# LewisClifton/Deep-Super-Resolution

Hardware: AMD Instinct MI355X
Metric: HR Mpixels/sec x4 GAN train step; PSNR delta vs reference (higher is better)
Workload: dtype bf16; 1 GPU; gan_x4: full GAN step x4 (G + D + VGG19 perceptual), batch 32/GPU, 128x128->512x512; global_batch=32, parallelism=dp1

## Files before the change

### deep-super-resolution_amd/csrc/conv_wgrad_tile.hip

```cpp
#include "dsr_common.h"
#include "dsr_kernels.h"

__device__ __forceinline__ s16x4 tr_read(const unsigned char* p) {
  return __builtin_amdgcn_ds_read_tr16_b64_v4i16((__attribute__((address_space(3))) s16x4*)(p));
}
__device__ __forceinline__ U4 tr_frag(const unsigned char* base, int p1, int p2, int chunk, int within) {
  s16x4 lo = tr_read(base + p1 * 128 + ((chunk ^ (p1 & 7)) << 4) + within);
  s16x4 hi = tr_read(base + p2 * 128 + ((chunk ^ (p2 & 7)) << 4) + within);
  return __builtin_bit_cast(U4, __builtin_shufflevector(lo, hi, 0, 1, 2, 3, 4, 5, 6, 7));
}

template <int DT, int KH, int KW, int S>
__global__ __launch_bounds__(256, 2) void conv_wgrad_tile_kernel(const WgradTileArgs a) {
  constexpr int R = (S == 1) ? 4 : 2;
  constexpr int HR = (R - 1) * S + KH, HC = 31 * S + KW;
  constexpr int NT = KH * KW;
  __shared__ __attribute__((aligned(16))) unsigned char sX[HR * HC * 128];
  __shared__ __attribute__((aligned(16))) unsigned char sY[R * 32 * 128];

  const int tid = threadIdx.x, lane = tid & 63, wave = __builtin_amdgcn_readfirstlane(tid >> 6);
  const int wr = wave >> 1, wc = wave & 1;
  const int g = lane >> 4, l16 = lane & 15, q4 = l16 >> 2, cc = 4 * (l16 & 3);
  const int pair = blockIdx.x;
  const int co0 = (pair / a.tiles_ci) * 64, ci0 = (pair % a.tiles_ci) * 64;
  const unsigned short* __restrict__ X = reinterpret_cast<const unsigned short*>(a.x);
  const unsigned short* __restrict__ DY = reinterpret_cast<const unsigned short*>(a.dy);

  f32x4 acc[NT][2][2];
#pragma unroll
  for (int t = 0; t < NT; ++t)
#pragma unroll
    for (int i = 0; i < 2; ++i)
#pragma unroll
      for (int j = 0; j < 2; ++j) acc[t][i][j] = f32x4{0.f, 0.f, 0.f, 0.f};

  const int c = tid & 7, pbase = tid >> 3;
  const bool yc_ok = (co0 + c * 8) < a.CoutP, xc_ok = (ci0 + c * 8) < a.CinP;
  int t_end = (blockIdx.y + 1) * a.tiles_per_block;
  if (t_end > a.ntiles) t_end = a.ntiles;
  const int per_img = a.tiles_y * a.tiles_x;

  for (int t = blockIdx.y * a.tiles_per_block; t < t_end; ++t) {
    const int n = t / per_img;
    const int rem = t - n * per_img;
    const int oy0 = (rem / a.tiles_x) * R, ox0 = (rem % a.tiles_x) * 32;
    __syncthreads();
#pragma unroll
    for (int i = 0; i < R * 32 * 8 / 256; ++i) {
      const int p = pbase + 32 * i;
      const int oy = oy0 + (p >> 5), ox = ox0 + (p & 31);
      const bool ok = yc_ok && oy < a.OH && ox < a.OW;
      U4 v = load16_or_zero(DY, ((size_t)(n * a.OH + oy) * a.OW + ox) * a.CoutP + co0 + c * 8, ok);
      *reinterpret_cast<U4*>(sY + p * 128 + ((c ^ (p & 7)) << 4)) = v;
    }
    {
      constexpr int NV = (HR * HC + 31) / 32;
      U4 v[NV];
#pragma unroll
      for (int u = 0; u < NV; ++u) {
        const int q = pbase + 32 * u;
        const int hr = q / HC, hc = q - hr * HC;
        bool ok = xc_ok && q < HR * HC;
        const int iy = pad_index(oy0 * S + hr - a.pad, a.IH, a.pad_mode, ok);
        const int ix = pad_index(ox0 * S + hc - a.pad, a.IW, a.pad_mode, ok);
        v[u] = load16_or_zero(X, ((size_t)(n * a.IH + iy) * a.IW + ix) * a.CinP + ci0 + c * 8, ok);
      }
#pragma unroll
      for (int u = 0; u < NV; ++u) {
        const int q = pbase + 32 * u;
        if (q < HR * HC) *reinterpret_cast<U4*>(sX + q * 128 + ((c ^ (q & 7)) << 4)) = v[u];
      }
    }
    __syncthreads();
#pragma unroll 1
    for (int r = 0; r < R; ++r) {
      U4 fa[2];
#pragma unroll
      for (int i = 0; i < 2; ++i) {
        const int ch = wr * 32 + i * 16 + cc;
        fa[i] = tr_frag(sY, r * 32 + 4 * g + q4, r * 32 + 16 + 4 * g + q4, ch >> 3, (ch & 7) * 2);
      }
#pragma unroll
      for (int kh = 0; kh < KH; ++kh)
#pragma unroll
        for (int kw = 0; kw < KW; ++kw) {
          const int qb = (r * S + kh) * HC + kw;
          const int q1 = qb + (4 * g + q4) * S, q2 = qb + (16 + 4 * g + q4) * S;
          U4 fb[2];
#pragma unroll
          for (int j = 0; j < 2; ++j) {
            const int ch = wc * 32 + j * 16 + cc;
            fb[j] = tr_frag(sX, q1, q2, ch >> 3, (ch & 7) * 2);
          }
#pragma unroll
          for (int i = 0; i < 2; ++i)
#pragma unroll
            for (int j = 0; j < 2; ++j) acc[kh * KW + kw][i][j] = mfma16<DT>(fa[i], fb[j], acc[kh * KW + kw][i][j]);
        }
    }
  }

  float* P = a.partial + (size_t)blockIdx.y * NT * a.CoutP * a.CinP;
#pragma unroll
  for (int t = 0; t < NT; ++t)
#pragma unroll
    for (int i = 0; i < 2; ++i)
#pragma unroll
      for (int j = 0; j < 2; ++j)
#pragma unroll
        for (int r = 0; r < 4; ++r) {
          const int co = co0 + wr * 32 + i * 16 + 4 * g + r, ci = ci0 + wc * 32 + j * 16 + l16;
          if (co < a.CoutP && ci < a.CinP) P[((size_t)t * a.CoutP + co) * a.CinP + ci] = acc[t][i][j][r];
        }
}

template <int DT>
__device__ __forceinline__ void conv_wgrad_dma_body(const WgradTileArgs& a, const int pair, const int ychunk) {
  constexpr int R = 2, HC = 40, HR = R + 2;
  constexpr int XB = HR * HC * 128, YB = R * 32 * 128, STAGE = XB + YB;
  __shared__ __attribute__((aligned(16))) unsigned char smem[2 * STAGE];

  const int tid = threadIdx.x, lane = tid & 63, wave = __builtin_amdgcn_readfirstlane(tid >> 6);
  const int g = lane >> 4, l16 = lane & 15, q4 = l16 >> 2, cc = 4 * (l16 & 3);
  const int co0 = (pair / a.tiles_ci) * 64, ci0 = (pair % a.tiles_ci) * 64;

  f32x4 acc[9][4];
#pragma unroll
  for (int t = 0; t < 9; ++t)
#pragma unroll
    for (int i = 0; i < 4; ++i) acc[t][i] = f32x4{0.f, 0.f, 0.f, 0.f};

  const int lp = 4 * g + q4;
  int offA[4], offB[3];
#pragma unroll
  for (int i = 0; i < 4; ++i) {
    const int ch = i * 16 + cc;
    offA[i] = XB + lp * 128 + (((ch >> 3) ^ (lp & 7)) << 4) + (ch & 7) * 2;
  }
#pragma unroll
  for (int kw = 0; kw < 3; ++kw) {
    const int ch = wave * 16 + cc;
    offB[kw] = lp * 128 + (((ch >> 3) ^ ((kw + lp) & 7)) << 4) + (ch & 7) * 2;
  }

  const int chunk = (tid & 7) ^ ((tid >> 3) & 7), pb = tid >> 3;
  const bool yc_ok = (co0 + chunk * 8) < a.CoutP, xc_ok = (ci0 + chunk * 8) < a.CinP;
  const BufSrd xrsrc = make_srd(const_cast<void*>(a.x), a.x_bytes);
  const BufSrd yrsrc = make_srd(const_cast<void*>(a.dy), a.dy_bytes);
  constexpr unsigned OOB = 0xFFFFFFF0u;
  typedef __attribute__((address_space(3))) void* lds_ptr;
  const int per_img = a.tiles_y * a.tiles_x;
  constexpr int NX = (HR * HC) / 32, NY = (R * 32) / 32;
  constexpr int FAR = 0x7FFFFF00;
  int xpart[NX], ypart[NY];
  unsigned hc_pack = 0;
#pragma unroll
  for (int u = 0; u < NX; ++u) {
    const int q = pb + 32 * u;
    const int hr = q / HC, hc = q - hr * HC;
    xpart[u] = (xc_ok && hc < 34) ? ((hr * a.IW + hc) * a.CinP + ci0 + chunk * 8) * 2 : FAR;
    hc_pack |= (unsigned)hc << (6 * u);
  }
#pragma unroll
  for (int u = 0; u < NY; ++u) {
    const int p = pb + 32 * u;
    ypart[u] = yc_ok ? (((p >> 5) * a.OW + (p & 31)) * a.CoutP + co0 + chunk * 8) * 2 : FAR;
  }
  const unsigned ximg = (unsigned)(a.IH * a.IW * a.CinP * 2), yimg = (unsigned)(a.OH * a.OW * a.CoutP * 2);
  const bool fast = a.pad_mode == DSR_PAD_ZERO;
  struct TileXY {
    int n, ty, tx;
  };
  auto dma = [&](const TileXY& tc, int buf) {
    const int n = tc.n;
    const int oy0 = tc.ty * R, ox0 = tc.tx * 32;
    unsigned char* st = smem + buf * STAGE;
    if (fast) {
      const BufSrd xr = make_srd(const_cast<unsigned char*>(reinterpret_cast<const unsigned char*>(a.x)) + (size_t)n * ximg, ximg);
      const BufSrd yr = make_srd(const_cast<unsigned char*>(reinterpret_cast<const unsigned char*>(a.dy)) + (size_t)n * yimg, yimg);
      const int xs = ((oy0 - a.pad) * a.IW + ox0 - a.pad) * a.CinP * 2;
      const int ys = (oy0 * a.OW + ox0) * a.CoutP * 2;
      unsigned char* dx = st + 8 * wave * 128;
      if (ox0 - a.pad >= 0 && ox0 - a.pad + 34 <= a.IW) {
#pragma unroll
        for (int u = 0; u < NX; ++u)
          lds_dma16(xr, dx + 32 * u * 128, (unsigned)(xpart[u] + xs));
      } else {
#pragma unroll
        for (int u = 0; u < NX; ++u) {
          const int ix = ox0 - a.pad + (int)((hc_pack >> (6 * u)) & 63);
          lds_dma16(xr, dx + 32 * u * 128, (unsigned)ix < (unsigned)a.IW ? (unsigned)(xpart[u] + xs) : OOB);
        }
      }
      if (ox0 + 32 <= a.OW) {
#pragma unroll
        for (int u = 0; u < NY; ++u)
          lds_dma16(yr, dx + XB + 32 * u * 128, (unsigned)(ypart[u] + ys));
      } else {
#pragma unroll
        for (int u = 0; u < NY; ++u)
          lds_dma16(yr, dx + XB + 32 * u * 128, ox0 + (pb & 31) < a.OW ? (unsigned)(ypart[u] + ys) : OOB);
      }
      return;
    }
#pragma unroll
    for (int u = 0; u < (HR * HC) / 32; ++u) {
      const int q = pb + 32 * u;
      const int hr = q / HC, hc = q - hr * HC;
      bool ok = xc_ok && hc < 34;
      const int iy = pad_index(oy0 + hr - a.pad, a.IH, a.pad_mode, ok);
      const int ix = pad_index(ox0 + hc - a.pad, a.IW, a.pad_mode, ok);
      lds_dma16(xrsrc, st + (32 * u + 8 * wave) * 128, ok ? (unsigned)((((n * a.IH + iy) * a.IW + ix) * a.CinP + ci0 + chunk * 8) * 2) : OOB);
    }
#pragma unroll
    for (int u = 0; u < (R * 32) / 32; ++u) {
      const int p = pb + 32 * u;
      const int oy = oy0 + (p >> 5), ox = ox0 + (p & 31);
      const bool ok = yc_ok && oy < a.OH && ox < a.OW;
      lds_dma16(yrsrc, st + XB + (32 * u + 8 * wave) * 128, ok ? (unsigned)((((n * a.OH + oy) * a.OW + ox) * a.CoutP + co0 + chunk * 8) * 2) : OOB);
    }
  };
  auto next_tile = [&](TileXY c) {
    if (++c.tx == a.tiles_x) {
      c.tx = 0;
      if (++c.ty == a.tiles_y) {
        c.ty = 0;
        ++c.n;
      }
    }
    return c;
  };

  int t = ychunk * a.tiles_per_block;
  int t_end = t + a.tiles_per_block;
  if (t_end > a.ntiles) t_end = a.ntiles;
  TileXY nxt;
  nxt.n = t / per_img;
  nxt.ty = (t - nxt.n * per_img) / a.tiles_x;
  nxt.tx = t - nxt.n * per_img - nxt.ty * a.tiles_x;
  __builtin_amdgcn_s_setprio(1);
  if (t < t_end) dma(nxt, 0);
  int buf = 0;
  for (; t < t_end; ++t, buf ^= 1) {
    asm volatile("s_waitcnt vmcnt(0)" ::: "memory");
    __builtin_amdgcn_s_barrier();
    asm volatile("" ::: "memory");
    nxt = next_tile(nxt);
    if (t + 1 < t_end) dma(nxt, buf ^ 1);
    __builtin_amdgcn_s_setprio(0);
    const unsigned char* st = smem + buf * STAGE;
    auto frag = [&](int off) {
      const s16x4 lo = tr_read(st + off);
      const s16x4 hi = tr_read(st + off + 2048);
      return __builtin_bit_cast(U4, __builtin_shufflevector(lo, hi, 0, 1, 2, 3, 4, 5, 6, 7));
    };
    constexpr int NU = 3 * HR;
    auto load_b = [&](int u) {
      const int kw = u / HR, h = u - kw * HR;
      return frag(offB[kw] + (h * HC + kw) * 128);
    };
    U4 fa[R][4], fb[3];
#pragma unroll
    for (int i = 0; i < 4; ++i) fa[0][i] = frag(offA[i]);
    fb[0] = load_b(0);
    fb[1] = load_b(1);
#pragma unroll
    for (int r = 1; r < R; ++r)
#pragma unroll
      for (int i = 0; i < 4; ++i) fa[r][i] = frag(offA[i] + r * 32 * 128);
#pragma unroll
    for (int u = 0; u < NU; ++u) {
      if (u + 2 < NU) fb[(u + 2) % 3] = load_b(u + 2);
      __builtin_amdgcn_sched_barrier(0);
      const int kw = u / HR, h = u - kw * HR;
#pragma unroll
      for (int r = 0; r < R; ++r) {
        const int kh = h - r;
        if (kh < 0 || kh > 2) continue;
#pragma unroll
        for (int i = 0; i < 4; ++i) acc[kh * 3 + kw][i] = mfma16<DT>(fa[r][i], fb[u % 3], acc[kh * 3 + kw][i]);
      }
      __builtin_amdgcn_sched_barrier(0);
    }
    __builtin_amdgcn_s_setprio(1);
  }

  float* P = a.partial + (size_t)ychunk * 9 * a.CoutP * a.CinP;
#pragma unroll
  for (int tp = 0; tp < 9; ++tp)
#pragma unroll
    for (int i = 0; i < 4; ++i)
#pragma unroll
      for (int r = 0; r < 4; ++r) {
        const int co = co0 + i * 16 + 4 * g + r, ci = ci0 + wave * 16 + l16;
        if (co < a.CoutP && ci < a.CinP) P[((size_t)tp * a.CoutP + co) * a.CinP + ci] = acc[tp][i][r];
      }
}

template <int DT>
__global__ __launch_bounds__(256, 2) void conv_wgrad_dma_kernel(const WgradTileArgs a) {
  conv_wgrad_dma_body<DT>(a, blockIdx.x, blockIdx.y);
}

template <int DT>
__global__ __launch_bounds__(256, 2) void conv_wgrad_dma_batch_kernel(const WgradBatchArgs b) {
  int pi = 0;
  while (pi + 1 < b.count && (int)blockIdx.x >= b.first_block[pi + 1]) ++pi;
  pi = __builtin_amdgcn_readfirstlane(pi);
  const WgradTileArgs a = b.p[pi];
  const int local = (int)blockIdx.x - b.first_block[pi];
  const int pairs = a.tiles_co * a.tiles_ci;
  conv_wgrad_dma_body<DT>(a, local % pairs, local / pairs);
}

template <int DT, int COH = 1>
__global__ __launch_bounds__(256 * COH, 2) void conv_wgrad_dma_s2_kernel(const WgradTileArgs a) {
  constexpr int HC = 80, HR = 3, NSLOT = HR * HC;
  constexpr int XB = NSLOT * 128, YB = 32 * 128, STAGE = XB + COH * YB;
  __shared__ __attribute__((aligned(16))) unsigned char smem[2 * STAGE];

  const int tid = threadIdx.x & 255, lane = tid & 63, wave = __builtin_amdgcn_readfirstlane((threadIdx.x >> 6) & 3);
  const int hsel = __builtin_amdgcn_readfirstlane(threadIdx.x >> 8);
  const int g = lane >> 4, l16 = lane & 15, q4 = l16 >> 2, cc = 4 * (l16 & 3);
  const int pair = blockIdx.x;
  const int co0 = (pair / a.tiles_ci) * 64 * COH + hsel * 64, ci0 = (pair % a.tiles_ci) * 64;

  f32x4 acc[9][4];
#pragma unroll
  for (int t = 0; t < 9; ++t)
#pragma unroll
    for (int i = 0; i < 4; ++i) acc[t][i] = f32x4{0.f, 0.f, 0.f, 0.f};

  const int lp = 4 * g + q4;
  int offA[4], offB[2];
#pragma unroll
  for (int i = 0; i < 4; ++i) {
    const int ch = i * 16 + cc;
    offA[i] = XB + hsel * YB + lp * 128 + (((ch >> 3) ^ (lp & 7)) << 4) + (ch & 7) * 2;
  }
#pragma unroll
  for (int v = 0; v < 2; ++v) {
    const int ch = wave * 16 + cc;
    offB[v] = 2 * lp * 128 + (((ch >> 3) ^ ((lp + v) & 7)) << 4) + (ch & 7) * 2;
  }

  const int pb = tid >> 3;
  const int xchunk = (tid & 7) ^ ((4 * wave + (lane >> 4)) & 7);
  const int ychunk = (tid & 7) ^ ((tid >> 3) & 7);
  const bool yc_ok = (co0 + ychunk * 8) < a.CoutP, xc_ok = (ci0 + xchunk * 8) < a.CinP;
  const BufSrd xrsrc = make_srd(const_cast<void*>(a.x), a.x_bytes);
  const BufSrd yrsrc = make_srd(const_cast<void*>(a.dy), a.dy_bytes);
  constexpr unsigned OOB = 0xFFFFFFF0u;
  typedef __attribute__((address_space(3))) void* lds_ptr;
  const int per_img = a.tiles_y * a.tiles_x;
  constexpr int NX = (NSLOT + 31) / 32;
  constexpr int FAR = 0x7FFFFF00;
  int xpart[NX];
  unsigned hc_lo = 0, hc_hi = 0;
#pragma unroll
  for (int u = 0; u < NX; ++u) {
    const int q = pb + 32 * u;
    const int hr = q / HC, hc = q - hr * HC;
    xpart[u] = (xc_ok && hc < 65 && hr < HR) ? ((hr * a.IW + hc) * a.CinP + ci0 + xchunk * 8) * 2 : FAR;
    if (u < 4) hc_lo |= (unsigned)hc << (7 * u);
    else hc_hi |= (unsigned)hc << (7 * (u - 4));
  }
  const int ypart = yc_ok ? (pb * a.CoutP + co0 + ychunk * 8) * 2 : FAR;
  const unsigned ximg = (unsigned)(a.IH * a.IW * a.CinP * 2), yimg = (unsigned)(a.OH * a.OW * a.CoutP * 2);
  const bool fast = a.pad_mode == DSR_PAD_ZERO;
  struct TileXY {
    int n, ty, tx;
  };
  auto dma = [&](const TileXY& tc, int buf) {
    const int n = tc.n, oy0 = tc.ty, ox0 = tc.tx * 32;
    unsigned char* st = smem + buf * STAGE;
    if (fast) {
      const BufSrd xr = make_srd(const_cast<unsigned char*>(reinterpret_cast<const unsigned char*>(a.x)) + (size_t)n * ximg, ximg);
      const BufSrd yr = make_srd(const_cast<unsigned char*>(reinterpret_cast<const unsigned char*>(a.dy)) + (size_t)n * yimg, yimg);
      const int ix0 = ox0 * 2 - a.pad;
      const int xs = ((oy0 * 2 - a.pad) * a.IW + ix0) * a.CinP * 2;
      const int ys = (oy0 * a.OW + ox0) * a.CoutP * 2;
      unsigned char* dx = st + 8 * wave * 128;
      const bool interior = ix0 >= 0 && ix0 + 65 <= a.IW;
#pragma unroll
      for (int u = 0; u < NX; ++u) {
        if (COH == 2 && (u & 1) != hsel) continue;
        if (32 * u + 8 * wave < NSLOT) {
          unsigned off = (unsigned)(xpart[u] + xs);
          if (!interior) {
            const int hc = (int)(((u < 4 ? hc_lo >> (7 * u) : hc_hi >> (7 * (u - 4)))) & 127);
            if (!((unsigned)(ix0 + hc) < (unsigned)a.IW)) off = OOB;
          }
          lds_dma16(xr, dx + 32 * u * 128, off);
        }
      }
      lds_dma16(yr, dx + XB + hsel * YB, (ox0 + 32 <= a.OW || ox0 + pb < a.OW) ? (unsigned)(ypart + ys) : OOB);
      return;
    }
#pragma unroll
    for (int u = 0; u < (NSLOT + 31) / 32; ++u) {
      if (COH == 2 && (u & 1) != hsel) continue;
      if (32 * u + 8 * wave < NSLOT) {
        const int q = pb + 32 * u;
        const int hr = q / HC, hc = q - hr * HC;
        bool ok = xc_ok && hc < 65;
        const int iy = pad_index(oy0 * 2 + hr - a.pad, a.IH, a.pad_mode, ok);
        const int ix = pad_index(ox0 * 2 + hc - a.pad, a.IW, a.pad_mode, ok);
        lds_dma16(xrsrc, st + (32 * u + 8 * wave) * 128, ok ? (unsigned)((((n * a.IH + iy) * a.IW + ix) * a.CinP + ci0 + xchunk * 8) * 2) : OOB);
      }
    }
    {
      const int ox = ox0 + pb;
      const bool ok = yc_ok && ox < a.OW;
      lds_dma16(yrsrc, st + XB + hsel * YB + 8 * wave * 128, ok ? (unsigned)((((n * a.OH + oy0) * a.OW + ox) * a.CoutP + co0 + ychunk * 8) * 2) : OOB);
    }
  };

  int t = blockIdx.y * a.tiles_per_block;
  int t_end = t + a.tiles_per_block;
  if (t_end > a.ntiles) t_end = a.ntiles;
  TileXY nxt;
  nxt.n = t / per_img;
  nxt.ty = (t - nxt.n * per_img) / a.tiles_x;
  nxt.tx = t - nxt.n * per_img - nxt.ty * a.tiles_x;
  __builtin_amdgcn_s_setprio(1);
  if (t < t_end) dma(nxt, 0);
  int buf = 0;
  for (; t < t_end; ++t, buf ^= 1) {
    asm volatile("s_waitcnt vmcnt(0)" ::: "memory");
    __builtin_amdgcn_s_barrier();
    asm volatile("" ::: "memory");
    if (++nxt.tx == a.tiles_x) {
      nxt.tx = 0;
      if (++nxt.ty == a.tiles_y) {
        nxt.ty = 0;
        ++nxt.n;
      }
    }
    if (t + 1 < t_end) dma(nxt, buf ^ 1);
    __builtin_amdgcn_s_setprio(0);
    const unsigned char* st = smem + buf * STAGE;
    U4 fa[4], fb[3];
    auto load_b = [&](int u) {
      const int kh = u / 3, kw = u % 3;
      const s16x4 lo = tr_read(st + offB[kw >> 1] + (kh * HC + kw) * 128);
      const s16x4 hi = tr_read(st + offB[kw >> 1] + (kh * HC + kw) * 128 + 32 * 128);
      return __builtin_bit_cast(U4, __builtin_shufflevector(lo, hi, 0, 1, 2, 3, 4, 5, 6, 7));
    };
#pragma unroll
    for (int i = 0; i < 4; ++i) {
      const s16x4 lo = tr_read(st + offA[i]);
      const s16x4 hi = tr_read(st + offA[i] + 2048);
      fa[i] = __builtin_bit_cast(U4, __builtin_shufflevector(lo, hi, 0, 1, 2, 3, 4, 5, 6, 7));
    }
    fb[0] = load_b(0);
    fb[1] = load_b(1);
#pragma unroll
    for (int u = 0; u < 9; ++u) {
      if (u + 2 < 9) fb[(u + 2) % 3] = load_b(u + 2);
      __builtin_amdgcn_sched_barrier(0);
#pragma unroll
      for (int i = 0; i < 4; ++i) acc[u][i] = mfma16<DT>(fa[i], fb[u % 3], acc[u][i]);
      __builtin_amdgcn_sched_barrier(0);
    }
    __builtin_amdgcn_s_setprio(1);
  }

  float* P = a.partial + (size_t)blockIdx.y * 9 * a.CoutP * a.CinP;
#pragma unroll
  for (int tp = 0; tp < 9; ++tp)
#pragma unroll
    for (int i = 0; i < 4; ++i)
#pragma unroll
      for (int r = 0; r < 4; ++r) {
        const int co = co0 + i * 16 + 4 * g + r, ci = ci0 + wave * 16 + l16;
        if (co < a.CoutP && ci < a.CinP) P[((size_t)tp * a.CoutP + co) * a.CinP + ci] = acc[tp][i][r];
      }
}

static bool dsr_wgrad_s2_co128(int KH, int stride, int CoutP, long long x_bytes) {
  const char* e = getenv("DSR_WGRAD_S2_CO128");
  const int mode = e ? atoi(e) : 1;
  if (mode == 0 || KH != 3 || stride != 2 || CoutP < 128 || CoutP % 128 != 0) return false;
  return mode == 2 || x_bytes >= 400ll * 1000 * 1000;
}

int dsr_wgrad_tile_plan(int KH, int KW, int stride, int N, int OH, int OW, int CinP, int CoutP, WgradTileArgs* a) {
  const bool k3 = KH == 3 && KW == 3 && (stride == 1 || stride == 2);
  const bool k1 = KH == 1 && KW == 1 && stride == 1;
  if (!k3 && !k1) return 0;
  const int R = k1 ? 4 : (stride == 1 ? 2 : 1);
  a->tiles_y = (OH + R - 1) / R;
  a->tiles_x = (OW + 31) / 32;
  a->ntiles = N * a->tiles_y * a->tiles_x;
  const bool co128 = dsr_wgrad_s2_co128(KH, stride, CoutP, (long long)N * (2 * OH) * (2 * OW) * CinP * 2);
  a->tiles_co = co128 ? CoutP / 128 : (CoutP + 63) / 64;
  a->tiles_ci = (CinP + 63) / 64;
  long long pairs = (long long)a->tiles_co * a->tiles_ci;
  long long want = ((co128 ? 256 : 512) + pairs - 1) / pairs;
  if (want > a->ntiles) want = a->ntiles;
  if (want < 1) want = 1;
  a->tiles_per_block = (int)((a->ntiles + want - 1) / want);
  return (a->ntiles + a->tiles_per_block - 1) / a->tiles_per_block;
}

template <int DT>
static void launch_dt(const WgradTileArgs& a, int KH, int stride, dim3 grid, hipStream_t st) {
  if (KH == 3 && stride == 1)
    hipLaunchKernelGGL((conv_wgrad_dma_kernel<DT>), grid, dim3(256), 0, st, a);
  else if (KH == 3 && a.tiles_co * 128 == a.CoutP && a.tiles_co * 64 != a.CoutP)
    hipLaunchKernelGGL((conv_wgrad_dma_s2_kernel<DT, 2>), grid, dim3(512), 0, st, a);
  else if (KH == 3)
    hipLaunchKernelGGL((conv_wgrad_dma_s2_kernel<DT>), grid, dim3(256), 0, st, a);
  else
    hipLaunchKernelGGL((conv_wgrad_tile_kernel<DT, 1, 1, 1>), grid, dim3(256), 0, st, a);
}

void dsr_launch_wgrad_dma_batch(const WgradBatchArgs& b, int dtype, hipStream_t st) {
  const int blocks = b.first_block[b.count];
  if (dtype == DSR_DTYPE_BF16)
    hipLaunchKernelGGL((conv_wgrad_dma_batch_kernel<DSR_DTYPE_BF16>), dim3(blocks), dim3(256), 0, st, b);
  else
    hipLaunchKernelGGL((conv_wgrad_dma_batch_kernel<DSR_DTYPE_F16>), dim3(blocks), dim3(256), 0, st, b);
}

void dsr_launch_wgrad_tile(const WgradTileArgs& a, int KH, int stride, int ychunks, int dtype, hipStream_t st) {
  dim3 grid(a.tiles_co * a.tiles_ci, ychunks);
  if (dtype == DSR_DTYPE_BF16)
    launch_dt<DSR_DTYPE_BF16>(a, KH, stride, grid, st);
  else
    launch_dt<DSR_DTYPE_F16>(a, KH, stride, grid, st);
}
```

Baseline: 246.3 HR Mpixels/s.

## Restructure stride-2 wgrad kernel into parity-split two-row tiles with fragment reuse

The stride-2 3x3 weight-gradient kernel now processes two output rows per tile. Its input halo is stored in LDS as four parity-split (even/odd row and column) planes, so each loaded B fragment serves several kernel taps across both rows. This cuts LDS halo traffic and transpose reads per MFMA. The 64-wide Cout variant now runs two independent 256-thread halves in one 512-thread block, each writing its own partial slab. The 128-wide Cout path is enabled whenever CoutP is a multiple of 128, no longer gated on input size. The change adds LDS per block (launch bounds drop to 1 block per CU) and doubles the number of partial slabs that must be reduced for the 64-wide case.

```diff
diff --git a/deep-super-resolution_amd/csrc/conv_wgrad_tile.hip b/deep-super-resolution_amd/csrc/conv_wgrad_tile.hip
--- a/deep-super-resolution_amd/csrc/conv_wgrad_tile.hip
+++ b/deep-super-resolution_amd/csrc/conv_wgrad_tile.hip
@@ -313,17 +313,38 @@
   conv_wgrad_dma_body<DT>(a, local % pairs, local / pairs);
 }
 
-template <int DT, int COH = 1>
-__global__ __launch_bounds__(256 * COH, 2) void conv_wgrad_dma_s2_kernel(const WgradTileArgs a) {
-  constexpr int HC = 80, HR = 3, NSLOT = HR * HC;
-  constexpr int XB = NSLOT * 128, YB = 32 * 128, STAGE = XB + COH * YB;
+namespace s2 {
+constexpr int NSLOT = 360, NGRP = NSLOT / 8;
+constexpr int PITCH[2] = {40, 32};
+constexpr int BASE[2][2] = {{0, 120}, {216, 296}};
+struct Slot {
+  int hr, hc;
+  bool valid;
+};
+__device__ __forceinline__ Slot slot(int q) {
+  const int rp = q >= BASE[1][0], cp = q >= (rp ? BASE[1][1] : BASE[0][1]);
+  const int pitch = cp ? PITCH[1] : PITCH[0];
+  const int rel = q - (rp ? (cp ? BASE[1][1] : BASE[1][0]) : (cp ? BASE[0][1] : BASE[0][0]));
+  const int j = rel / pitch, k = rel - j * pitch;
+  return {2 * j + rp, 2 * k + cp, k < 33 - cp};
+}
+}
+
+template <int DT, int COH>
+__global__ __launch_bounds__(512, 1) void conv_wgrad_dma_s2_kernel(const WgradTileArgs a) {
+  constexpr int XB = s2::NSLOT * 128, YB = 2 * 32 * 128, STAGE = XB + COH * YB;
+  constexpr int NR = COH == 2 ? 2 : 1;
+  constexpr int HRU = 2 * NR + 1;
+  constexpr int NX = (s2::NGRP + 7) / 8;
+  constexpr int NY = COH == 2 ? 2 : 1;
   __shared__ __attribute__((aligned(16))) unsigned char smem[2 * STAGE];
 
-  const int tid = threadIdx.x & 255, lane = tid & 63, wave = __builtin_amdgcn_readfirstlane((threadIdx.x >> 6) & 3);
-  const int hsel = __builtin_amdgcn_readfirstlane(threadIdx.x >> 8);
+  const int tid = threadIdx.x, lane = tid & 63;
+  const int w8 = __builtin_amdgcn_readfirstlane(tid >> 6);
+  const int wave = w8 & 3, hsel = w8 >> 2;
+  const int row0 = COH == 2 ? 0 : hsel;
   const int g = lane >> 4, l16 = lane & 15, q4 = l16 >> 2, cc = 4 * (l16 & 3);
-  const int pair = blockIdx.x;
-  const int co0 = (pair / a.tiles_ci) * 64 * COH + hsel * 64, ci0 = (pair % a.tiles_ci) * 64;
+  const int co0 = (blockIdx.x / a.tiles_ci) * 64 * COH + (COH == 2 ? hsel * 64 : 0), ci0 = (blockIdx.x % a.tiles_ci) * 64;
 
   f32x4 acc[9][4];
 #pragma unroll
@@ -332,87 +353,95 @@
     for (int i = 0; i < 4; ++i) acc[t][i] = f32x4{0.f, 0.f, 0.f, 0.f};
 
   const int lp = 4 * g + q4;
-  int offA[4], offB[2];
+  int offA[4], offB[3];
 #pragma unroll
   for (int i = 0; i < 4; ++i) {
     const int ch = i * 16 + cc;
-    offA[i] = XB + hsel * YB + lp * 128 + (((ch >> 3) ^ (lp & 7)) << 4) + (ch & 7) * 2;
-  }
-#pragma unroll
-  for (int v = 0; v < 2; ++v) {
-    const int ch = wave * 16 + cc;
-    offB[v] = 2 * lp * 128 + (((ch >> 3) ^ ((lp + v) & 7)) << 4) + (ch & 7) * 2;
-  }
-
-  const int pb = tid >> 3;
-  const int xchunk = (tid & 7) ^ ((4 * wave + (lane >> 4)) & 7);
-  const int ychunk = (tid & 7) ^ ((tid >> 3) & 7);
-  const bool yc_ok = (co0 + ychunk * 8) < a.CoutP, xc_ok = (ci0 + xchunk * 8) < a.CinP;
+    offA[i] = XB + (COH == 2 ? hsel * YB : row0 * 32 * 128) + lp * 128 + (((ch >> 3) ^ (lp & 7)) << 4) + (ch & 7) * 2;
+  }
+#pragma unroll
+  for (int kw = 0; kw < 3; ++kw) {
+    const int ch = wave * 16 + cc, q = lp + (kw == 2);
+    offB[kw] = (row0 * s2::PITCH[kw == 1] + q) * 128 + (((ch >> 3) ^ (q & 7)) << 4) + (ch & 7) * 2;
+  }
+
+  const int chunk = (lane & 7) ^ (lane >> 3);
+  const bool yc_ok = (co0 + chunk * 8) < a.CoutP, xc_ok = (ci0 + chunk * 8) < a.CinP;
   const BufSrd xrsrc = make_srd(const_cast<void*>(a.x), a.x_bytes);
   const BufSrd yrsrc = make_srd(const_cast<void*>(a.dy), a.dy_bytes);
   constexpr unsigned OOB = 0xFFFFFFF0u;
-  typedef __attribute__((address_space(3))) void* lds_ptr;
+  constexpr int FAR = 0x7FFFFF00;
   const int per_img = a.tiles_y * a.tiles_x;
-  constexpr int NX = (NSLOT + 31) / 32;
-  constexpr int FAR = 0x7FFFFF00;
-  int xpart[NX];
+  auto ygroup = [&](int v) { return COH == 2 ? wave + 4 * v : w8; };
+  int xpart[NX], ypart[NY];
   unsigned hc_lo = 0, hc_hi = 0;
 #pragma unroll
   for (int u = 0; u < NX; ++u) {
-    const int q = pb + 32 * u;
-    const int hr = q / HC, hc = q - hr * HC;
-    xpart[u] = (xc_ok && hc < 65 && hr < HR) ? ((hr * a.IW + hc) * a.CinP + ci0 + xchunk * 8) * 2 : FAR;
-    if (u < 4) hc_lo |= (unsigned)hc << (7 * u);
-    else hc_hi |= (unsigned)hc << (7 * (u - 4));
-  }
-  const int ypart = yc_ok ? (pb * a.CoutP + co0 + ychunk * 8) * 2 : FAR;
+    const int s = 8 * u + w8;
+    const s2::Slot sl = s2::slot(8 * (s < s2::NGRP ? s : 0) + (lane >> 3));
+    xpart[u] = (xc_ok && sl.valid) ? ((sl.hr * a.IW + sl.hc) * a.CinP + ci0 + chunk * 8) * 2 : FAR;
+    if (u < 4) hc_lo |= (unsigned)sl.hc << (7 * u);
+    else hc_hi |= (unsigned)sl.hc << (7 * (u - 4));
+  }
+#pragma unroll
+  for (int v = 0; v < NY; ++v) {
+    const int p = 8 * ygroup(v) + (lane >> 3);
+    ypart[v] = yc_ok ? (((p >> 5) * a.OW + (p & 31)) * a.CoutP + co0 + chunk * 8) * 2 : FAR;
+  }
   const unsigned ximg = (unsigned)(a.IH * a.IW * a.CinP * 2), yimg = (unsigned)(a.OH * a.OW * a.CoutP * 2);
   const bool fast = a.pad_mode == DSR_PAD_ZERO;
   struct TileXY {
     int n, ty, tx;
   };
   auto dma = [&](const TileXY& tc, int buf) {
-    const int n = tc.n, oy0 = tc.ty, ox0 = tc.tx * 32;
+    const int n = tc.n, oy0 = tc.ty * 2, ox0 = tc.tx * 32;
     unsigned char* st = smem + buf * STAGE;
+    unsigned char* sy = st + XB + (COH == 2 ? hsel * YB : 0);
     if (fast) {
       const BufSrd xr = make_srd(const_cast<unsigned char*>(reinterpret_cast<const unsigned char*>(a.x)) + (size_t)n * ximg, ximg);
       const BufSrd yr = make_srd(const_cast<unsigned char*>(reinterpret_cast<const unsigned char*>(a.dy)) + (size_t)n * yimg, yimg);
       const int ix0 = ox0 * 2 - a.pad;
       const int xs = ((oy0 * 2 - a.pad) * a.IW + ix0) * a.CinP * 2;
       const int ys = (oy0 * a.OW + ox0) * a.CoutP * 2;
-      unsigned char* dx = st + 8 * wave * 128;
       const bool interior = ix0 >= 0 && ix0 + 65 <= a.IW;
 #pragma unroll
       for (int u = 0; u < NX; ++u) {
-        if (COH == 2 && (u & 1) != hsel) continue;
-        if (32 * u + 8 * wave < NSLOT) {
-          unsigned off = (unsigned)(xpart[u] + xs);
+        const int s = 8 * u + w8;
+        if (s < s2::NGRP) {
+          unsigned off = (unsigned)xpart[u] + (unsigned)xs;
           if (!interior) {
             const int hc = (int)(((u < 4 ? hc_lo >> (7 * u) : hc_hi >> (7 * (u - 4)))) & 127);
             if (!((unsigned)(ix0 + hc) < (unsigned)a.IW)) off = OOB;
           }
-          lds_dma16(xr, dx + 32 * u * 128, off);
+          lds_dma16(xr, st + s * 1024, off);
         }
       }
-      lds_dma16(yr, dx + XB + hsel * YB, (ox0 + 32 <= a.OW || ox0 + pb < a.OW) ? (unsigned)(ypart + ys) : OOB);
+      const bool yfull = ox0 + 32 <= a.OW;
+#pragma unroll
+      for (int v = 0; v < NY; ++v) {
+        const int grp = ygroup(v);
+        const bool ok = yfull || ox0 + ((8 * grp + (lane >> 3)) & 31) < a.OW;
+        lds_dma16(yr, sy + grp * 1024, ok ? (unsigned)ypart[v] + (unsigned)ys : OOB);
+      }
       return;
     }
 #pragma unroll
-    for (int u = 0; u < (NSLOT + 31) / 32; ++u) {
-      if (COH == 2 && (u & 1) != hsel) continue;
-      if (32 * u + 8 * wave < NSLOT) {
-        const int q = pb + 32 * u;
-        const int hr = q / HC, hc = q - hr * HC;
-        bool ok = xc_ok && hc < 65;
-        const int iy = pad_index(oy0 * 2 + hr - a.pad, a.IH, a.pad_mode, ok);
-        const int ix = pad_index(ox0 * 2 + hc - a.pad, a.IW, a.pad_mode, ok);
-        lds_dma16(xrsrc, st + (32 * u + 8 * wave) * 128, ok ? (unsigned)((((n * a.IH + iy) * a.IW + ix) * a.CinP + ci0 + xchunk * 8) * 2) : OOB);
-      }
-    }
-    {
-      const int ox = ox0 + pb;
-      const bool ok = yc_ok && ox < a.OW;
-      lds_dma16(yrsrc, st + XB + hsel * YB + 8 * wave * 128, ok ? (unsigned)((((n * a.OH + oy0) * a.OW + ox) * a.CoutP + co0 + ychunk * 8) * 2) : OOB);
+    for (int u = 0; u < NX; ++u) {
+      const int s = 8 * u + w8;
+      if (s < s2::NGRP) {
+        const s2::Slot sl = s2::slot(8 * s + (lane >> 3));
+        bool ok = xc_ok && sl.valid;
+        const int iy = pad_index(oy0 * 2 + sl.hr - a.pad, a.IH, a.pad_mode, ok);
+        const int ix = pad_index(ox0 * 2 + sl.hc - a.pad, a.IW, a.pad_mode, ok);
+        lds_dma16(xrsrc, st + s * 1024, ok ? (unsigned)((((n * a.IH + iy) * a.IW + ix) * a.CinP + ci0 + chunk * 8) * 2) : OOB);
+      }
+    }
+#pragma unroll
+    for (int v = 0; v < NY; ++v) {
+      const int grp = ygroup(v), p = 8 * grp + (lane >> 3);
+      const int oy = oy0 + (p >> 5), ox = ox0 + (p & 31);
+      const bool ok = yc_ok && oy < a.OH && ox < a.OW;
+      lds_dma16(yrsrc, sy + grp * 1024, ok ? (unsigned)((((n * a.OH + oy) * a.OW + ox) * a.CoutP + co0 + chunk * 8) * 2) : OOB);
     }
   };
 
@@ -440,33 +469,44 @@
     if (t + 1 < t_end) dma(nxt, buf ^ 1);
     __builtin_amdgcn_s_setprio(0);
     const unsigned char* st = smem + buf * STAGE;
-    U4 fa[4], fb[3];
-    auto load_b = [&](int u) {
-      const int kh = u / 3, kw = u % 3;
-      const s16x4 lo = tr_read(st + offB[kw >> 1] + (kh * HC + kw) * 128);
-      const s16x4 hi = tr_read(st + offB[kw >> 1] + (kh * HC + kw) * 128 + 32 * 128);
+    auto frag = [&](int off) {
+      const s16x4 lo = tr_read(st + off);
+      const s16x4 hi = tr_read(st + off + 2048);
       return __builtin_bit_cast(U4, __builtin_shufflevector(lo, hi, 0, 1, 2, 3, 4, 5, 6, 7));
     };
-#pragma unroll
-    for (int i = 0; i < 4; ++i) {
-      const s16x4 lo = tr_read(st + offA[i]);
-      const s16x4 hi = tr_read(st + offA[i] + 2048);
-      fa[i] = __builtin_bit_cast(U4, __builtin_shufflevector(lo, hi, 0, 1, 2, 3, 4, 5, 6, 7));
-    }
+    constexpr int NU = 3 * HRU;
+    auto load_b = [&](int u) {
+      const int kw = u / HRU, h = u - kw * HRU;
+      return frag(offB[kw] + (s2::BASE[h & 1][kw == 1] + (h >> 1) * s2::PITCH[kw == 1]) * 128);
+    };
+    U4 fa[NR][4], fb[3];
+#pragma unroll
+    for (int i = 0; i < 4; ++i) fa[0][i] = frag(offA[i]);
     fb[0] = load_b(0);
     fb[1] = load_b(1);
 #pragma unroll
-    for (int u = 0; u < 9; ++u) {
-      if (u + 2 < 9) fb[(u + 2) % 3] = load_b(u + 2);
+    for (int r = 1; r < NR; ++r)
+#pragma unroll
+      for (int i = 0; i < 4; ++i) fa[r][i] = frag(offA[i] + r * 32 * 128);
+#pragma unroll
+    for (int u = 0; u < NU; ++u) {
+      if (u + 2 < NU) fb[(u + 2) % 3] = load_b(u + 2);
       __builtin_amdgcn_sched_barrier(0);
-#pragma unroll
-      for (int i = 0; i < 4; ++i) acc[u][i] = mfma16<DT>(fa[i], fb[u % 3], acc[u][i]);
+      const int kw = u / HRU, h = u - kw * HRU;
+#pragma unroll
+      for (int r = 0; r < NR; ++r) {
+        const int kh = h - 2 * r;
+        if (kh < 0 || kh > 2) continue;
+#pragma unroll
+        for (int i = 0; i < 4; ++i) acc[kh * 3 + kw][i] = mfma16<DT>(fa[r][i], fb[u % 3], acc[kh * 3 + kw][i]);
+      }
       __builtin_amdgcn_sched_barrier(0);
     }
     __builtin_amdgcn_s_setprio(1);
   }
 
-  float* P = a.partial + (size_t)blockIdx.y * 9 * a.CoutP * a.CinP;
+  const int slab = COH == 2 ? blockIdx.y : 2 * blockIdx.y + hsel;
+  float* P = a.partial + (size_t)slab * 9 * a.CoutP * a.CinP;
 #pragma unroll
   for (int tp = 0; tp < 9; ++tp)
 #pragma unroll
@@ -478,40 +518,41 @@
       }
 }
 
-static bool dsr_wgrad_s2_co128(int KH, int stride, int CoutP, long long x_bytes) {
+static bool dsr_wgrad_s2_co128(int CoutP) {
   const char* e = getenv("DSR_WGRAD_S2_CO128");
-  const int mode = e ? atoi(e) : 1;
-  if (mode == 0 || KH != 3 || stride != 2 || CoutP < 128 || CoutP % 128 != 0) return false;
-  return mode == 2 || x_bytes >= 400ll * 1000 * 1000;
+  return !(e && atoi(e) == 0) && CoutP % 128 == 0;
 }
 
 int dsr_wgrad_tile_plan(int KH, int KW, int stride, int N, int OH, int OW, int CinP, int CoutP, WgradTileArgs* a) {
   const bool k3 = KH == 3 && KW == 3 && (stride == 1 || stride == 2);
   const bool k1 = KH == 1 && KW == 1 && stride == 1;
   if (!k3 && !k1) return 0;
-  const int R = k1 ? 4 : (stride == 1 ? 2 : 1);
+  const bool s2 = k3 && stride == 2;
+  const int R = k1 ? 4 : 2;
   a->tiles_y = (OH + R - 1) / R;
   a->tiles_x = (OW + 31) / 32;
   a->ntiles = N * a->tiles_y * a->tiles_x;
-  const bool co128 = dsr_wgrad_s2_co128(KH, stride, CoutP, (long long)N * (2 * OH) * (2 * OW) * CinP * 2);
+  const bool co128 = s2 && dsr_wgrad_s2_co128(CoutP);
   a->tiles_co = co128 ? CoutP / 128 : (CoutP + 63) / 64;
   a->tiles_ci = (CinP + 63) / 64;
   long long pairs = (long long)a->tiles_co * a->tiles_ci;
-  long long want = ((co128 ? 256 : 512) + pairs - 1) / pairs;
+  long long want = ((s2 ? 256 : 512) + pairs - 1) / pairs;
   if (want > a->ntiles) want = a->ntiles;
   if (want < 1) want = 1;
   a->tiles_per_block = (int)((a->ntiles + want - 1) / want);
-  return (a->ntiles + a->tiles_per_block - 1) / a->tiles_per_block;
+  const int chunks = (a->ntiles + a->tiles_per_block - 1) / a->tiles_per_block;
+  return s2 && !co128 ? 2 * chunks : chunks;
 }
 
 template <int DT>
-static void launch_dt(const WgradTileArgs& a, int KH, int stride, dim3 grid, hipStream_t st) {
+static void launch_dt(const WgradTileArgs& a, int KH, int stride, int ychunks, hipStream_t st) {
+  const dim3 grid(a.tiles_co * a.tiles_ci, ychunks);
   if (KH == 3 && stride == 1)
     hipLaunchKernelGGL((conv_wgrad_dma_kernel<DT>), grid, dim3(256), 0, st, a);
-  else if (KH == 3 && a.tiles_co * 128 == a.CoutP && a.tiles_co * 64 != a.CoutP)
+  else if (KH == 3 && a.tiles_co * 128 == a.CoutP)
     hipLaunchKernelGGL((conv_wgrad_dma_s2_kernel<DT, 2>), grid, dim3(512), 0, st, a);
   else if (KH == 3)
-    hipLaunchKernelGGL((conv_wgrad_dma_s2_kernel<DT>), grid, dim3(256), 0, st, a);
+    hipLaunchKernelGGL((conv_wgrad_dma_s2_kernel<DT, 1>), dim3(grid.x, ychunks / 2), dim3(512), 0, st, a);
   else
     hipLaunchKernelGGL((conv_wgrad_tile_kernel<DT, 1, 1, 1>), grid, dim3(256), 0, st, a);
 }
@@ -525,9 +566,8 @@
 }
 
 void dsr_launch_wgrad_tile(const WgradTileArgs& a, int KH, int stride, int ychunks, int dtype, hipStream_t st) {
-  dim3 grid(a.tiles_co * a.tiles_ci, ychunks);
   if (dtype == DSR_DTYPE_BF16)
-    launch_dt<DSR_DTYPE_BF16>(a, KH, stride, grid, st);
+    launch_dt<DSR_DTYPE_BF16>(a, KH, stride, ychunks, st);
   else
-    launch_dt<DSR_DTYPE_F16>(a, KH, stride, grid, st);
-}
+    launch_dt<DSR_DTYPE_F16>(a, KH, stride, ychunks, st);
+}
```

Result: no change. 248.7 HR Mpixels/s, median of 6 (+1.0%).
